# brade31919/radar_depth

Hardware: AMD Instinct MI355X
Metric: training samples/sec, resnet18_latefusion b=16 450x800 rgbd, 1/2/4/8 MI355X (higher is better)
Workload: dtype f32

## Files before the change

radar_depth_amd/csrc/layout.hip:

```cpp
#include "common.h"

namespace rd {

__device__ __forceinline__ int64_t packed_index(int quad, int64_t t, int64_t rows, int64_t row, int64_t ldc, int64_t col) {
    return quad ? ((t * (rows >> 2) + (row >> 2)) * ldc + col) * 4 + (row & 3) : (t * rows + row) * ldc + col;
}
__device__ __forceinline__ int64_t packed_index_bf16(int64_t t, int64_t rows, int64_t row, int64_t ldc, int64_t col) {
    return ((t * (rows >> 3) + (row >> 3)) * ldc + col) * 8 + (row & 7);
}
__global__ void pack_weights_kernel(const float* __restrict__ w, float* __restrict__ packed, int O, int I, int T,
                                    int ldc, int off, int rows_total, int transpose) {
    const int64_t total = (int64_t)O * I * T;
    for (int64_t e = (int64_t)blockIdx.x * blockDim.x + threadIdx.x; e < total; e += (int64_t)gridDim.x * blockDim.x) {
        int t, o, i;
        if (!transpose) {
            o = (int)(e % O);
            const int64_t r = e / O;
            i = (int)(r % I);
            t = (int)(r / I);
            packed[packed_index(1, t, I, i, ldc, off + o)] = w[((int64_t)o * I + i) * T + t];
        } else {
            i = (int)(e % I);
            const int64_t r = e / I;
            o = (int)(r % O);
            t = (int)(r / O);
            packed[packed_index(1, t, rows_total, off + o, ldc, i)] = w[((int64_t)o * I + i) * T + t];
        }
    }
}

__global__ void pack_weights_bf16_kernel(const float* __restrict__ w, __bf16* __restrict__ packed, int O, int I, int T,
                                         int ldc, int off, int rows_total, int transpose) {
    const int64_t total = (int64_t)O * I * T;
    for (int64_t e = (int64_t)blockIdx.x * blockDim.x + threadIdx.x; e < total; e += (int64_t)gridDim.x * blockDim.x) {
        const int o = (int)(e % O);
        const int64_t r = e / O;
        const int i = (int)(r % I), t = (int)(r / I);
        const float v = w[((int64_t)o * I + i) * T + t];
        if (!transpose) packed[packed_index_bf16(t, I, i, ldc, off + o)] = (__bf16)v;
        else packed[packed_index_bf16(t, rows_total, off + o, ldc, i)] = (__bf16)v;
    }
}

struct PackJob {
    const float* src;
    float* dst;
    const float* scale;
    int O, I, T, ldc, off, rows_total, transpose, first_block;
    int quad;
    int scale_col;
};
__device__ __forceinline__ void store_split3(__bf16* dst, int64_t idx, int64_t plane, float v) {
    const __bf16 h = (__bf16)v;
    float r = v - (float)h;
    const __bf16 m = (__bf16)r;
    r -= (float)m;
    dst[idx] = h;
    dst[idx + plane] = m;
    dst[idx + 2 * plane] = (__bf16)r;
}
constexpr int PACK_CHUNK = 2048;
__device__ __forceinline__ void pack_units_bf16(const PackJob& j, int64_t u) {
    const int R = j.transpose ? j.O : j.I;
    const int Cn = j.transpose ? j.I : j.O;
    const int64_t units = (int64_t)(R >> 3) * Cn;
    if (u >= units) return;
    const int col = (int)(u % Cn), r8 = (int)(u / Cn);
    const int rows_total = j.transpose ? j.rows_total : j.I;
    const int row0 = (j.transpose ? j.off : 0) + r8 * 8, colp = (j.transpose ? 0 : j.off) + col;
    __bf16* dst = reinterpret_cast<__bf16*>(j.dst);
    const int64_t plane = (int64_t)j.T * rows_total * j.ldc;
    for (int t = 0; t < j.T; ++t) {
        float v[8];
#pragma unroll
        for (int r = 0; r < 8; ++r) {
            const int o = j.transpose ? r8 * 8 + r : col, i = j.transpose ? col : r8 * 8 + r;
            v[r] = j.src[((int64_t)o * j.I + i) * j.T + t];
            if (j.scale) v[r] *= j.scale[j.scale_col ? i : o];
        }
        const int64_t idx = packed_index_bf16(t, rows_total, row0, j.ldc, colp);
        unsigned w0[4], w1[4], w2[4];
#pragma unroll
        for (int q = 0; q < 4; ++q) {
            float a = v[2 * q], b = v[2 * q + 1];
            w0[q] = cvt_pk_bf16(a, b);
            a -= __uint_as_float(w0[q] << 16); b -= __uint_as_float(w0[q] & 0xffff0000u);
            w1[q] = cvt_pk_bf16(a, b);
            a -= __uint_as_float(w1[q] << 16); b -= __uint_as_float(w1[q] & 0xffff0000u);
            w2[q] = cvt_pk_bf16(a, b);
        }
        *reinterpret_cast<uint4*>(dst + idx) = make_uint4(w0[0], w0[1], w0[2], w0[3]);
        if (j.quad == 3) {
            *reinterpret_cast<uint4*>(dst + idx + plane) = make_uint4(w1[0], w1[1], w1[2], w1[3]);
            *reinterpret_cast<uint4*>(dst + idx + 2 * plane) = make_uint4(w2[0], w2[1], w2[2], w2[3]);
        }
    }
}
__global__ __launch_bounds__(256) void pack_weights_batched_kernel(const PackJob* __restrict__ jobs, const int* __restrict__ block_job) {
    const PackJob j = jobs[block_job[blockIdx.x]];
    if (j.quad >= 2 && ((j.transpose ? (j.O | j.off | j.rows_total) : j.I) & 7) == 0) {
        pack_units_bf16(j, (int64_t)(blockIdx.x - j.first_block) * 256 + threadIdx.x);
        return;
    }
    const int64_t total = (int64_t)j.O * j.I * j.T;
    const int64_t base = (int64_t)(blockIdx.x - j.first_block) * PACK_CHUNK;
#pragma unroll
    for (int u = 0; u < PACK_CHUNK / 256; ++u) {
        const int64_t e64 = base + u * 256 + threadIdx.x;
        if (e64 >= total) break;
        const unsigned e = (unsigned)e64;
        if (!j.transpose) {
            const unsigned r = e / (unsigned)j.O;
            const int o = (int)(e - r * (unsigned)j.O);
            const int t = (int)(r / (unsigned)j.I), i = (int)(r - (r / (unsigned)j.I) * (unsigned)j.I);
            float v = j.src[((int64_t)o * j.I + i) * j.T + t];
            if (j.scale) v *= j.scale[j.scale_col ? i : o];
            if (j.quad == 3) store_split3(reinterpret_cast<__bf16*>(j.dst), packed_index_bf16(t, j.I, i, j.ldc, j.off + o), (int64_t)j.T * j.I * j.ldc, v);
            else if (j.quad == 2) reinterpret_cast<__bf16*>(j.dst)[packed_index_bf16(t, j.I, i, j.ldc, j.off + o)] = (__bf16)v;
            else j.dst[packed_index(j.quad, t, j.I, i, j.ldc, j.off + o)] = v;
        } else {
            const unsigned r = e / (unsigned)j.I;
            const int i = (int)(e - r * (unsigned)j.I);
            const int t = (int)(r / (unsigned)j.O), o = (int)(r - (r / (unsigned)j.O) * (unsigned)j.O);
            float v = j.src[((int64_t)o * j.I + i) * j.T + t];
            if (j.scale) v *= j.scale[j.scale_col ? i : o];
            if (j.quad == 3) store_split3(reinterpret_cast<__bf16*>(j.dst), packed_index_bf16(t, j.rows_total, j.off + o, j.ldc, i), (int64_t)j.T * j.rows_total * j.ldc, v);
            else if (j.quad == 2) reinterpret_cast<__bf16*>(j.dst)[packed_index_bf16(t, j.rows_total, j.off + o, j.ldc, i)] = (__bf16)v;
            else j.dst[packed_index(j.quad, t, j.rows_total, j.off + o, j.ldc, i)] = v;
        }
    }
}

__global__ void fill_kernel(float* __restrict__ p, int64_t n, float v) {
    for (int64_t e = (int64_t)blockIdx.x * blockDim.x + threadIdx.x; e < n; e += (int64_t)gridDim.x * blockDim.x) p[e] = v;
}

__global__ void transpose_kernel(const float* __restrict__ src, float* __restrict__ dst, int rows, int cols) {
    __shared__ float tile[32][33];
    const int n = blockIdx.z;
    src += (size_t)n * rows * cols;
    dst += (size_t)n * rows * cols;
    const int c0 = blockIdx.x * 32, r0 = blockIdx.y * 32;
    for (int j = threadIdx.y; j < 32; j += blockDim.y) {
        const int r = r0 + j, c = c0 + threadIdx.x;
        if (r < rows && c < cols) tile[j][threadIdx.x] = src[(size_t)r * cols + c];
    }
    rd_sync();
    for (int j = threadIdx.y; j < 32; j += blockDim.y) {
        const int c = c0 + j, r = r0 + threadIdx.x;
        if (r < rows && c < cols) dst[(size_t)c * rows + r] = tile[threadIdx.x][j];
    }
}

static int grid_for(int64_t n, int block) {
// ... 81 lines not shown
```

radar_depth_amd/csrc/wgrad.hip:

```cpp
#include <stdlib.h>

#include <mutex>
#include <string>
#include <type_traits>
#include <unordered_map>
#include <vector>

#include "common.h"

namespace rd {

template <int B, int E, int ST, typename F>
__device__ __forceinline__ void static_for(F&& f) {
    if constexpr (B < E) {
        f(std::integral_constant<int, B>{});
        static_for<B + ST, E, ST>(f);
    }
}

constexpr int WG_MAX_TG = 9;
constexpr int WG_MAX_GROUPS = 5;
constexpr int WG_MAX_PIX = 512;
constexpr int WG_PITCH = 27;

struct WgTapGroup {
    int n;
    int8_t dh[WG_MAX_TG], dw[WG_MAX_TG], oh[WG_MAX_TG], ow[WG_MAX_TG];
    int16_t widx[WG_MAX_TG];
};

struct WgradArgs {
    const float* in;
    const float* dout;
    float* slabs;
    int N, Hi, Wi, Cin, ldi, Ho, Wo, Cout, ldo, IS, OS;
    int lh, lw, TH, TW, tiles_h, tiles_w, total_tiles, tiles_per_split, n_splits;
    int dh_min, dh_max, dw_min, dw_max;
    int n_cib, n_cob, n_tg;
    int S;
    int compact, off_h, off_w;
    int debug;
    WgTapGroup tg[WG_MAX_GROUPS];
};

template <int TG, int MF, bool LAYOUT_A, bool SHB, int PITCH, int RW>
__global__ __launch_bounds__(256) __attribute__((amdgpu_waves_per_eu(2))) void wgrad_kernel(const WgradArgs a) {
    constexpr int CIB = LAYOUT_A ? 64 : MF;
    constexpr int COB = LAYOUT_A ? 64 : MF;
    constexpr int KP = MF == 32 ? 2 : 4;
    constexpr int WLP = LAYOUT_A ? 1 : 4;
    constexpr int NACC = MF == 32 ? 16 : 4;
    extern __shared__ __attribute__((aligned(16))) float smem[];
    const int tid = threadIdx.x, lane = tid & 63, wave = tid >> 6;
    const int lm = lane & (MF - 1), lk = lane / MF;
    const int wci = LAYOUT_A ? (wave >> 1) : 0, wco = LAYOUT_A ? (wave & 1) : 0;
    const int wpix = LAYOUT_A ? 0 : wave;

    const int vid = xcd_remap(blockIdx.x, gridDim.x);
    const int n_groups = a.n_cib * a.n_cob * a.n_tg;
    const int g = vid % n_groups, split = vid / n_groups;
    const int tgi = g % a.n_tg;
// ... 300 lines not shown
            _Pragma("unroll") for (int t = 0; t < TG; ++t) acc[t] = __builtin_amdgcn_mfma_f32_32x32x2f32(AV[t], BV, acc[t], 0, 0, 0);
#define RD_WS_SCHED()                                                                              \
            _Pragma("unroll") for (int i = 0; i < TG; ++i) {                                           \
                __builtin_amdgcn_sched_group_barrier(0x008, 1, 0);                                     \
                __builtin_amdgcn_sched_group_barrier(0x100, 1, 0);                                     \
            }                                                                                          \
            __builtin_amdgcn_sched_barrier(0);
            RD_WS_LOAD(a0, b0, 0)
            __builtin_amdgcn_sched_barrier(0);
            static_for<0, 2 * STEPS, 2>([&](auto sc) {
                constexpr int S = decltype(sc)::value;
                RD_WS_LOAD(a1, b1, S + 1)
                RD_WS_MFMA(a0, b0)
                RD_WS_SCHED()
                if constexpr (S + 2 < 2 * STEPS) { RD_WS_LOAD(a0, b0, S + 2) }
                RD_WS_MFMA(a1, b1)
                RD_WS_SCHED()
            });
#undef RD_WS_LOAD
#undef RD_WS_MFMA
#undef RD_WS_SCHED
        }
    }

    float* slab = a.slabs + (size_t)split * a.S * a.Cin * a.Cout;
    const int co = cob0 + wco * 32 + lm;
#pragma unroll
    for (int t = 0; t < TG; ++t) {
        float* dst = slab + (size_t)G.widx[t] * a.Cin * a.Cout;
#pragma unroll
        for (int i = 0; i < 16; ++i) {
            const int ci = cib0 + wci * 32 + (i & 3) + 8 * (i >> 2) + 4 * lk;
            if (ci < a.Cin && co < a.Cout) dst[(size_t)ci * a.Cout + co] = acc[t][i];
        }
    }
}

__global__ __launch_bounds__(256) void wgrad_reduce1_kernel(const float* __restrict__ slabs, float* __restrict__ tmp,
                                                            int n_splits, int J, int64_t E4) {
    const int j = blockIdx.y;
    const float4* src = reinterpret_cast<const float4*>(slabs);
    float4* dst = reinterpret_cast<float4*>(tmp);
    for (int64_t e = (int64_t)blockIdx.x * blockDim.x + threadIdx.x; e < E4; e += (int64_t)gridDim.x * blockDim.x) {
        float4 s = make_float4(0.f, 0.f, 0.f, 0.f);
#pragma unroll 4
        for (int k = j; k < n_splits; k += J) {
            const float4 v = src[(int64_t)k * E4 + e];
            s.x += v.x; s.y += v.y; s.z += v.z; s.w += v.w;
        }
        dst[(int64_t)j * E4 + e] = s;
    }
}

__global__ __launch_bounds__(256) void wgrad_reduce2_kernel(const float* __restrict__ tmp, float* __restrict__ grad, int J,
                                                            int64_t E, int S, int Cin, int Cout, int O, int I, int co_off,
                                                            int accumulate) {
    const int64_t total = (int64_t)S * I * O;
    const bool small = total < (1ll << 31);
    for (int64_t e = (int64_t)blockIdx.x * blockDim.x + threadIdx.x; e < total; e += (int64_t)gridDim.x * blockDim.x) {
        int o, i, t;
        if (small) {
            const unsigned u = (unsigned)e, r = u / (unsigned)O;
            o = (int)(u - r * (unsigned)O);
            t = (int)(r / (unsigned)I);
            i = (int)(r - (unsigned)t * (unsigned)I);
        } else {
            o = (int)(e % O);
            const int64_t r = e / O;
            i = (int)(r % I);
            t = (int)(r / I);
        }
        const float* src = tmp + ((int64_t)t * Cin + i) * Cout + co_off + o;
        float s = 0.f;
        for (int k = 0; k < J; ++k) s += src[k * E];
        float* dst = grad + ((int64_t)o * I + i) * S + t;
        *dst = accumulate ? *dst + s : s;
    }
}

int launch_slab_reduce(const float* slabs, int n_splits, int64_t E, float* tmp, float* grad_oihw, int S, int Cin, int Cout,
                       int O, int I, int co_off, int accumulate, hipStream_t s) {
    RD_CHECK_ARG(E % 4 == 0, "slab_reduce: slab size must be a multiple of 4");
    const int J = n_splits < 16 ? n_splits : 16;
    const int64_t E4 = E / 4;
    if (n_splits <= 16) tmp = const_cast<float*>(slabs);
    else if (co_off == 0) {
        int64_t g1 = cdiv64(E4, 256);
        if (g1 > 2048) g1 = 2048;
        hipLaunchKernelGGL(wgrad_reduce1_kernel, dim3((int)g1, J), dim3(256), 0, s, slabs, tmp, n_splits, J, E4);
        RD_CHECK_LAUNCH("wgrad_reduce1_kernel");
    }
    const int64_t total = (int64_t)S * I * O;
    int64_t g = cdiv64(total, 256);
    if (g > 4096) g = 4096;
    hipLaunchKernelGGL(wgrad_reduce2_kernel, dim3((int)g), dim3(256), 0, s, tmp, grad_oihw, J, E, S, Cin, Cout, O, I, co_off,
                       accumulate);
    RD_CHECK_LAUNCH("wgrad_reduce2_kernel");
    return RD_OK;
}

__global__ __launch_bounds__(256) void wgrad_reduce1_batched_kernel(const RdReduceJob* __restrict__ jobs, const int32_t* __restrict__ block_job) {
    const RdReduceJob jb = jobs[block_job[blockIdx.x]];
    const int lb = (int)blockIdx.x - jb.first_block1;
    const int J = jb.J, j = lb % J, bx = lb / J, nbx = jb.n_blocks1 / J;
    const int64_t E4 = jb.E / 4;
    const float4* src = reinterpret_cast<const float4*>(jb.slabs);
    float4* dst = reinterpret_cast<float4*>(jb.tmp);
    for (int64_t e = (int64_t)bx * 256 + threadIdx.x; e < E4; e += (int64_t)nbx * 256) {
        float4 s = make_float4(0.f, 0.f, 0.f, 0.f);
#pragma unroll 4
        for (int k = j; k < jb.n_splits; k += J) {
            const float4 v = src[(int64_t)k * E4 + e];
            s.x += v.x; s.y += v.y; s.z += v.z; s.w += v.w;
        }
        dst[(int64_t)j * E4 + e] = s;
    }
}

__global__ __launch_bounds__(256) void wgrad_reduce2_batched_kernel(const RdReduceJob* __restrict__ jobs, const int32_t* __restrict__ block_job) {
    const RdReduceJob jb = jobs[block_job[blockIdx.x]];
    const int lb = (int)blockIdx.x - jb.first_block2;
    const unsigned total = (unsigned)jb.S * (unsigned)jb.I * (unsigned)jb.O;
    const float* tmp = jb.n_splits <= 16 ? jb.slabs : jb.tmp;
    for (unsigned u = (unsigned)lb * 256u + threadIdx.x; u < total; u += (unsigned)jb.n_blocks2 * 256u) {
        const unsigned r = u / (unsigned)jb.O;
        const int o = (int)(u - r * (unsigned)jb.O);
        const int t = (int)(r / (unsigned)jb.I);
        const int i = (int)(r - (unsigned)t * (unsigned)jb.I);
        const float* src = tmp + ((int64_t)t * jb.Cin + i) * jb.Cout + jb.co_off + o;
        float s = 0.f;
        for (int k = 0; k < jb.J; ++k) s += src[k * jb.E];
        float* dst = jb.grad + ((int64_t)o * jb.I + i) * jb.S + t;
        *dst = jb.accumulate ? *dst + s : s;
    }
}

int make_reduce_job(const float* slabs, int n_splits, int64_t E, float* grad_oihw, int S, int Cin, int Cout, int O, int I, int co_off,
                    int accumulate, RdReduceJob* jb) {
    RD_CHECK_ARG(E % 4 == 0, "slab_reduce: slab size must be a multiple of 4");
    RD_CHECK_ARG((int64_t)S * I * O < (1ll << 31), "wgrad_reduce_job: one weight tensor must stay below 2^31 elements");
    const int J = n_splits < 16 ? n_splits : 16;
    jb->slabs = slabs; jb->tmp = const_cast<float*>(slabs) + (int64_t)n_splits * E; jb->grad = grad_oihw;
    jb->E = E; jb->n_splits = n_splits; jb->J = J; jb->S = S; jb->Cin = Cin; jb->Cout = Cout; jb->O = O; jb->I = I;
    jb->co_off = co_off; jb->accumulate = accumulate;
    int64_t g1 = cdiv64(E / 4, 256);
    if (g1 > 2048) g1 = 2048;
    jb->n_blocks1 = (n_splits > 16 && co_off == 0) ? (int)g1 * J : 0;
    int64_t g2 = cdiv64((int64_t)S * I * O, 256);
    if (g2 > 4096) g2 = 4096;
    jb->n_blocks2 = (int)g2;
    jb->first_block1 = jb->first_block2 = 0;
    jb->pad_ = 0;
    return RD_OK;
}

struct WgradPlan {
    int TG, MF, layoutA;
    int TH, TW, tiles_h, tiles_w, total_tiles, tiles_per_split, n_splits, slab_splits;
    int n_cib, n_cob, n_tg, S, J, shb;
    int pitch;
    int rw;
    int per_phase;
    int strip;
    int w16;
    int w1x1;
    WgradStripArgs sa;
    size_t lds;
};

static inline bool tile_is_tiled(const struct WgradPlan* tile);
static int plan_wgrad(const RdConvDesc& d_in, WgradPlan& pl, WgradArgs* out, int ph = -1, const WgradPlan* tile = nullptr) {
    RdConvDesc d = d_in;
    int S_all = 0;
    for (int i = 0; i < d_in.n_phases; ++i)
        for (int t = 0; t < d_in.phase[i].n_taps; ++t) S_all = S_all > d_in.phase[i].widx[t] + 1 ? S_all : d_in.phase[i].widx[t] + 1;
    if (ph >= 0) {
        d.n_phases = 1;
        d.phase[0] = d_in.phase[ph];
    }
    const RdPhase& P0 = d.phase[0];
    int ntaps = 0, S = 0;
    int dh_min = 127, dh_max = -127, dw_min = 127, dw_max = -127;
    for (int i = 0; i < d.n_phases; ++i) {
        const RdPhase& p = d.phase[i];
        RD_CHECK_ARG(p.lh == P0.lh && p.lw == P0.lw, "wgrad: phases must share one logical grid");
        ntaps += p.n_taps;
        for (int t = 0; t < p.n_taps; ++t) S = S > p.widx[t] + 1 ? S : p.widx[t] + 1;
        dh_min = dh_min < p.dh_min ? dh_min : p.dh_min;
        dh_max = dh_max > p.dh_max ? dh_max : p.dh_max;
        dw_min = dw_min < p.dw_min ? dw_min : p.dw_min;
        dw_max = dw_max > p.dw_max ? dw_max : p.dw_max;
    }
    S = S_all;
// ... 371 lines not shown
```

radar_depth_amd/csrc/wino_split.hip:

```cpp
#include <stdlib.h>

#include <type_traits>

#include "common.h"

namespace rd {

typedef __bf16 wbf16x8 __attribute__((ext_vector_type(8)));
typedef unsigned int wu32x4 __attribute__((ext_vector_type(4)));
typedef float wf32x2 __attribute__((ext_vector_type(2)));
typedef __bf16 wbf16x2 __attribute__((ext_vector_type(2)));

constexpr int WN_TBH = 4, WN_TBW = 8;
constexpr int WN_T = WN_TBH * WN_TBW;
constexpr int WN_CB = 64;
constexpr int WN_AH = 16 * 3 * 2 * 512;
constexpr int WN_BH = 16 * 3 * 2 * 1024;
constexpr int WN_BUF = WN_AH;
constexpr int WN_ZP = 68;
constexpr unsigned WN_OOB = 0x80000000u;

struct WinoArgs {
    const float* in;
    const unsigned short* u;
// ... 239 lines not shown
            const float4 xv = ld4(a.bnb_x + px * a.bnb_ld + co);
            const float gx = y.x * act_grad_from_out(fmaf(bS.x, xv.x, bT.x), a.bnb_act), gy = y.y * act_grad_from_out(fmaf(bS.y, xv.y, bT.y), a.bnb_act);
            const float gz = y.z * act_grad_from_out(fmaf(bS.z, xv.z, bT.z), a.bnb_act), gw = y.w * act_grad_from_out(fmaf(bS.w, xv.w, bT.w), a.bnb_act);
            ssum.x += gx; ssum.y += gy; ssum.z += gz; ssum.w += gw;
            ssq.x += gx * (xv.x - bM.x); ssq.y += gy * (xv.y - bM.y); ssq.z += gz * (xv.z - bM.z); ssq.w += gw * (xv.w - bM.w);
        } else {
            ssum.x += y.x; ssum.y += y.y; ssum.z += y.z; ssum.w += y.w;
            ssq.x += y.x * y.x; ssq.y += y.y * y.y; ssq.z += y.z * y.z; ssq.w += y.w * y.w;
        }
    };
#pragma unroll
    for (int it = 0; it < 2; ++it) {
        const int rt = (tid >> 4) + 32 * it;
        const int m = rt >> 1, r = rt & 1;
        float4 z[4];
#pragma unroll
        for (int j = 0; j < 4; ++j) z[j] = *reinterpret_cast<const float4*>(zb + ((j * 2 + r) * WN_T + m) * WN_ZP + c4 * 4);
        float4 y0 = make_float4(z[0].x + z[1].x + z[2].x, z[0].y + z[1].y + z[2].y, z[0].z + z[1].z + z[2].z, z[0].w + z[1].w + z[2].w);
        float4 y1 = make_float4(z[1].x - z[2].x - z[3].x, z[1].y - z[2].y - z[3].y, z[1].z - z[2].z - z[3].z, z[1].w - z[2].w - z[3].w);
        const int oy = 2 * (by * WN_TBH + (m >> 3)) + r, ox = 2 * (bx * WN_TBW + (m & 7));
        const bool okr = oy < a.H && co < a.Cout;
        const bool ok0 = okr && ox < a.W, ok1 = okr && ox + 1 < a.W;
        const size_t pix = ((size_t)n * a.H + oy) * a.W + ox;
        if (a.addend) {
            if (ok0) { const float4 v = ld4(a.addend + pix * a.ld_add + co); y0.x += v.x; y0.y += v.y; y0.z += v.z; y0.w += v.w; }
            if (ok1) { const float4 v = ld4(a.addend + (pix + 1) * a.ld_add + co); y1.x += v.x; y1.y += v.y; y1.z += v.z; y1.w += v.w; }
        }
        if (ok0) {
            st4(a.out + pix * a.ldo + co, y0);
            if (a.stat) account(y0, pix);
        }
        if (ok1) {
            st4(a.out + (pix + 1) * a.ldo + co, y1);
            if (a.stat) account(y1, pix + 1);
        }
    }
    if (a.stat) {
        rd_sync();
        float* red = reinterpret_cast<float*>(wsm);
        const int row = tid >> 4;
        *reinterpret_cast<float4*>(red + (row * 2 + 0) * 64 + c4 * 4) = ssum;
        *reinterpret_cast<float4*>(red + (row * 2 + 1) * 64 + c4 * 4) = ssq;
        rd_sync();
        if (tid < 128) {
            const int which = tid >> 6, j = tid & 63;
            float s = 0.f;
#pragma unroll 8
            for (int rw = 0; rw < 32; ++rw) s += red[(rw * 2 + which) * 64 + j];
            if (cot * WN_CB + j < a.Cout) a.stat[((size_t)pt * (bnb ? 3 : 2) + which) * a.Cout + cot * WN_CB + j] = s;
        }
    }
}

__device__ __forceinline__ void wino_pack_body(const float* __restrict__ w, int O, int I, int flip, unsigned short* __restrict__ u, int e) {
    const int R = flip ? O : I, Q = flip ? I : O;
    const int r8n = R >> 3;
    if (e >= Q * r8n) return;
    const int q = e / r8n, r8 = e - q * r8n;
    const int nck = R >> 4;
    const int cot = q >> 6, ql = q & 63;
    const int chunk = r8 >> 1, kh8 = r8 & 1;
    unsigned short pc[16][3][8];
#pragma unroll
    for (int k = 0; k < 8; ++k) {
        const int r = r8 * 8 + k;
        const float* g = flip ? w + ((size_t)r * I + q) * 9 : w + ((size_t)q * I + r) * 9;
        double gg[3][3];
#pragma unroll
        for (int y = 0; y < 3; ++y)
#pragma unroll
            for (int x = 0; x < 3; ++x) gg[y][x] = flip ? (double)g[(2 - y) * 3 + (2 - x)] : (double)g[y * 3 + x];
        double t[4][3];
#pragma unroll
        for (int x = 0; x < 3; ++x) {
            t[0][x] = gg[0][x];
            t[1][x] = 0.5 * (gg[0][x] + gg[1][x] + gg[2][x]);
            t[2][x] = 0.5 * (gg[0][x] - gg[1][x] + gg[2][x]);
            t[3][x] = gg[2][x];
        }
#pragma unroll
        for (int i = 0; i < 4; ++i) {
            const double uu[4] = {t[i][0], 0.5 * (t[i][0] + t[i][1] + t[i][2]), 0.5 * (t[i][0] - t[i][1] + t[i][2]), t[i][2]};
#pragma unroll
            for (int j = 0; j < 4; ++j) {
                float f = (float)uu[j];
                const __bf16 p0 = (__bf16)uu[j];
                f -= (float)p0;
                const __bf16 p1 = (__bf16)f;
                f -= (float)p1;
                const __bf16 p2 = (__bf16)f;
                pc[i * 4 + j][0][k] = __builtin_bit_cast(unsigned short, p0);
                pc[i * 4 + j][1][k] = __builtin_bit_cast(unsigned short, p1);
                pc[i * 4 + j][2][k] = __builtin_bit_cast(unsigned short, p2);
            }
        }
    }
#pragma unroll
    for (int i = 0; i < 4; ++i)
#pragma unroll
        for (int j = 0; j < 4; ++j)
#pragma unroll
            for (int p = 0; p < 3; ++p) {
                const size_t o = ((size_t)cot * nck + chunk) * WN_BH + (((i * 4 + j) * 3 + p) * 2 + kh8) * 1024 + ql * 16;
                uint4 v;
                v.x = pc[i * 4 + j][p][0] | ((unsigned)pc[i * 4 + j][p][1] << 16);
                v.y = pc[i * 4 + j][p][2] | ((unsigned)pc[i * 4 + j][p][3] << 16);
                v.z = pc[i * 4 + j][p][4] | ((unsigned)pc[i * 4 + j][p][5] << 16);
                v.w = pc[i * 4 + j][p][6] | ((unsigned)pc[i * 4 + j][p][7] << 16);
                *reinterpret_cast<uint4*>(reinterpret_cast<char*>(u) + o) = v;
            }
}

__global__ __launch_bounds__(256) void wino_pack_kernel(const float* __restrict__ w, int O, int I, int flip, unsigned short* __restrict__ u) {
    wino_pack_body(w, O, I, flip, u, blockIdx.x * blockDim.x + threadIdx.x);
}

struct WinoPackJob {
    const float* w;
    unsigned short* u;
    int32_t O, I, flip, first_block;
};
__global__ __launch_bounds__(256) void wino_pack_batched_kernel(const WinoPackJob* __restrict__ jobs, const int32_t* __restrict__ block_job) {
    const WinoPackJob j = jobs[block_job[blockIdx.x]];
    wino_pack_body(j.w, j.O, j.I, j.flip, j.u, (blockIdx.x - j.first_block) * blockDim.x + threadIdx.x);
}

static bool wino_shape_ok(int H, int W, int Cin, int Cout, int ldi, int ldo) {
    return H >= 2 && W >= 2 && Cin >= 64 && Cin % 16 == 0 && Cout >= 64 && Cout % 64 == 0 && ldi % 4 == 0 && ldo % 4 == 0 &&
           (long long)H * W * ldi * 4 < 0x7fffffffll;
}
}

extern "C" int64_t rd_wino_packed_bytes(int32_t O, int32_t I, int32_t flip) {
    const int R = flip ? O : I, Q = flip ? I : O;
    return (int64_t)((Q + 63) / 64) * (R / 16) * rd::WN_BH;
}

extern "C" int rd_wino_pack(const float* w_oihw, int32_t O, int32_t I, int32_t flip, void* u_packed, void* stream) {
    RD_CHECK_ARG(w_oihw && u_packed && O > 0 && I > 0, "rd_wino_pack: bad arguments");
    const int R = flip ? O : I, Q = flip ? I : O;
    RD_CHECK_ARG(R % 16 == 0 && Q % 64 == 0, "rd_wino_pack: reduction channels %d %% 16, output channels %d %% 64", R, Q);
    const int n = Q * (R / 8);
    hipLaunchKernelGGL(rd::wino_pack_kernel, dim3((n + 255) / 256), dim3(256), 0, static_cast<hipStream_t>(stream), w_oihw, O, I, flip,
                       static_cast<unsigned short*>(u_packed));
    RD_CHECK_LAUNCH("wino_pack_kernel");
    return RD_OK;
}

extern "C" int rd_wino_pack_blocks(int32_t O, int32_t I, int32_t flip) {
    const int R = flip ? O : I, Q = flip ? I : O;
    return (Q * (R / 8) + 255) / 256;
}
extern "C" int rd_wino_pack_batched(const void* jobs, const int32_t* block_job, int32_t n_blocks, void* stream) {
    RD_CHECK_ARG(jobs && block_job && n_blocks > 0, "rd_wino_pack_batched: bad arguments");
    static_assert(sizeof(rd::WinoPackJob) == 32, "job record layout");
    hipLaunchKernelGGL(rd::wino_pack_batched_kernel, dim3(n_blocks), dim3(256), 0, static_cast<hipStream_t>(stream),
                       static_cast<const rd::WinoPackJob*>(jobs), block_job);
    RD_CHECK_LAUNCH("wino_pack_batched_kernel");
    return RD_OK;
}

extern "C" int rd_wino_preferred(int32_t H, int32_t W, int32_t Cin, int32_t Cout, int32_t ldi, int32_t ldo) {
    if (!rd::wino_shape_ok(H, W, Cin, Cout, ldi, ldo)) return 0;
    static const char* env = getenv("RD_WINO");
    if (env && !strcmp(env, "0")) return 0;
    if (env && !strcmp(env, "all")) return 1;
    return (Cin >= 512 || ((long long)H * W <= 1536 && Cin <= 128)) ? 1 : 0;
}

extern "C" int rd_wino_supported(int32_t H, int32_t W, int32_t Cin, int32_t Cout, int32_t ldi, int32_t ldo) {
    return rd::wino_shape_ok(H, W, Cin, Cout, ldi, ldo) ? 1 : 0;
}

extern "C" int rd_wino_stat_tiles(int32_t N, int32_t H, int32_t W) {
    const int th = (H + 1) / 2, tw = (W + 1) / 2;
    return N * ((th + rd::WN_TBH - 1) / rd::WN_TBH) * ((tw + rd::WN_TBW - 1) / rd::WN_TBW);
}
// ... 52 lines not shown
```

Before: 1103.

## Stage OIHW weight reads and gradient writes through LDS for coalesced access

Weight packing, the Winograd weight pack and the weight-gradient slab reduction now stage contiguous OIHW runs through shared memory tiles instead of scattered per-element global loads and stores. Reads and writes become vectorised float4 runs along the contiguous dimension, and a shared tile-shape helper picks tile sizes per tap count. This targets the uncoalesced memory traffic in the per-step weight packing and wgrad finalisation, at the cost of extra block barriers, LDS use and more complex boundary handling.

```diff
diff --git a/radar_depth_amd/csrc/layout.hip b/radar_depth_amd/csrc/layout.hip
--- a/radar_depth_amd/csrc/layout.hip
+++ b/radar_depth_amd/csrc/layout.hip
@@ -1,4 +1,5 @@
 #include "common.h"
+#include "oihw_tiles.h"
 
 namespace rd {
 
@@ -60,46 +61,79 @@
     dst[idx + 2 * plane] = (__bf16)r;
 }
 constexpr int PACK_CHUNK = 2048;
-__device__ __forceinline__ void pack_units_bf16(const PackJob& j, int64_t u) {
-    const int R = j.transpose ? j.O : j.I;
+__device__ __forceinline__ void pack_units_bf16(const PackJob& j, const PackTile& pt, int lb, int nb, float* lds) {
+#pragma clang fp contract(off)
+    const int tid = threadIdx.x;
+    const int R8 = (j.transpose ? j.O : j.I) >> 3;
     const int Cn = j.transpose ? j.I : j.O;
-    const int64_t units = (int64_t)(R >> 3) * Cn;
-    if (u >= units) return;
-    const int col = (int)(u % Cn), r8 = (int)(u / Cn);
+    const int n_ct = (Cn + pt.co - 1) / pt.co, n_kt = (R8 + pt.k8 - 1) / pt.k8;
     const int rows_total = j.transpose ? j.rows_total : j.I;
-    const int row0 = (j.transpose ? j.off : 0) + r8 * 8, colp = (j.transpose ? 0 : j.off) + col;
     __bf16* dst = reinterpret_cast<__bf16*>(j.dst);
     const int64_t plane = (int64_t)j.T * rows_total * j.ldc;
-    for (int t = 0; t < j.T; ++t) {
-        float v[8];
-#pragma unroll
-        for (int r = 0; r < 8; ++r) {
-            const int o = j.transpose ? r8 * 8 + r : col, i = j.transpose ? col : r8 * 8 + r;
-            v[r] = j.src[((int64_t)o * j.I + i) * j.T + t];
-            if (j.scale) v[r] *= j.scale[j.scale_col ? i : o];
-        }
-        const int64_t idx = packed_index_bf16(t, rows_total, row0, j.ldc, colp);
-        unsigned w0[4], w1[4], w2[4];
-#pragma unroll
-        for (int q = 0; q < 4; ++q) {
-            float a = v[2 * q], b = v[2 * q + 1];
-            w0[q] = cvt_pk_bf16(a, b);
-            a -= __uint_as_float(w0[q] << 16); b -= __uint_as_float(w0[q] & 0xffff0000u);
-            w1[q] = cvt_pk_bf16(a, b);
-            a -= __uint_as_float(w1[q] << 16); b -= __uint_as_float(w1[q] & 0xffff0000u);
-            w2[q] = cvt_pk_bf16(a, b);
-        }
-        *reinterpret_cast<uint4*>(dst + idx) = make_uint4(w0[0], w0[1], w0[2], w0[3]);
-        if (j.quad == 3) {
-            *reinterpret_cast<uint4*>(dst + idx + plane) = make_uint4(w1[0], w1[1], w1[2], w1[3]);
-            *reinterpret_cast<uint4*>(dst + idx + 2 * plane) = make_uint4(w2[0], w2[1], w2[2], w2[3]);
+    const int T = j.T, LP = pt.lp;
+    for (int tile = lb; tile < n_ct * n_kt; tile += nb) {
+        if (tile != lb) rd_sync();
+        const int kt = tile / n_ct, ct = tile - kt * n_ct;
+        const int c0 = ct * pt.co, u0 = kt * pt.k8;
+        const int cn = Cn - c0 < pt.co ? Cn - c0 : pt.co, kn = R8 - u0 < pt.k8 ? R8 - u0 : pt.k8;
+        const int n_runs = j.transpose ? kn * 8 : cn, len = j.transpose ? cn * T : kn * 8 * T;
+        const int nq = (len + 6) >> 2;
+        for (int idx = tid; idx < n_runs * nq; idx += 256) {
+            const int r = idx / nq, q = idx - r * nq;
+            const float* run = j.src + (j.transpose ? ((int64_t)(u0 * 8 + r) * j.I + c0) * T : ((int64_t)(c0 + r) * j.I + u0 * 8) * T);
+            const int a = (int)((reinterpret_cast<uintptr_t>(run) >> 2) & 3);
+            const int c = 4 * q - a;
+            if (c >= len) continue;
+            float* l = lds + r * LP + c;
+            if (c >= 0 && c + 4 <= len) {
+                const float4 v = *reinterpret_cast<const float4*>(run + c);
+                l[0] = v.x; l[1] = v.y; l[2] = v.z; l[3] = v.w;
+            } else {
+#pragma unroll
+                for (int e = 0; e < 4; ++e)
+                    if (c + e >= 0 && c + e < len) l[e] = run[c + e];
+            }
+        }
+        rd_sync();
+        for (int item = tid; item < cn * kn * T; item += 256) {
+            const int col = item % cn, kt_ = item / cn;
+            const int k = kt_ / T, t = kt_ - k * T;
+            float v[8];
+#pragma unroll
+            for (int r = 0; r < 8; ++r) {
+                v[r] = j.transpose ? lds[(k * 8 + r) * LP + col * T + t] : lds[col * LP + (k * 8 + r) * T + t];
+                if (j.scale) {
+                    const int o = j.transpose ? (u0 + k) * 8 + r : c0 + col, i = j.transpose ? c0 + col : (u0 + k) * 8 + r;
+                    v[r] *= j.scale[j.scale_col ? i : o];
+                }
+            }
+            const int row0 = (j.transpose ? j.off : 0) + (u0 + k) * 8, colp = (j.transpose ? 0 : j.off) + c0 + col;
+            const int64_t idx = packed_index_bf16(t, rows_total, row0, j.ldc, colp);
+            unsigned w0[4], w1[4], w2[4];
+#pragma unroll
+            for (int q = 0; q < 4; ++q) {
+                float a = v[2 * q], b = v[2 * q + 1];
+                w0[q] = cvt_pk_bf16(a, b);
+                a -= __uint_as_float(w0[q] << 16); b -= __uint_as_float(w0[q] & 0xffff0000u);
+                w1[q] = cvt_pk_bf16(a, b);
+                a -= __uint_as_float(w1[q] << 16); b -= __uint_as_float(w1[q] & 0xffff0000u);
+                w2[q] = cvt_pk_bf16(a, b);
+            }
+            *reinterpret_cast<uint4*>(dst + idx) = make_uint4(w0[0], w0[1], w0[2], w0[3]);
+            if (j.quad == 3) {
+                *reinterpret_cast<uint4*>(dst + idx + plane) = make_uint4(w1[0], w1[1], w1[2], w1[3]);
+                *reinterpret_cast<uint4*>(dst + idx + 2 * plane) = make_uint4(w2[0], w2[1], w2[2], w2[3]);
+            }
         }
     }
 }
 __global__ __launch_bounds__(256) void pack_weights_batched_kernel(const PackJob* __restrict__ jobs, const int* __restrict__ block_job) {
+    __shared__ float lds[PACK_LDS];
     const PackJob j = jobs[block_job[blockIdx.x]];
-    if (j.quad >= 2 && ((j.transpose ? (j.O | j.off | j.rows_total) : j.I) & 7) == 0) {
-        pack_units_bf16(j, (int64_t)(blockIdx.x - j.first_block) * 256 + threadIdx.x);
+    const PackTile pt = pack_tile(j.T, j.transpose);
+    if (j.quad >= 2 && ((j.transpose ? (j.O | j.off | j.rows_total) : j.I) & 7) == 0 && pt.co > 0) {
+        const int nb = (int)(((int64_t)j.O * j.I * j.T + PACK_CHUNK - 1) / PACK_CHUNK);
+        pack_units_bf16(j, pt, (int)(blockIdx.x - j.first_block), nb, lds);
         return;
     }
     const int64_t total = (int64_t)j.O * j.I * j.T;
diff --git a/radar_depth_amd/csrc/oihw_tiles.h b/radar_depth_amd/csrc/oihw_tiles.h
--- /dev/null
+++ b/radar_depth_amd/csrc/oihw_tiles.h
@@ -0,0 +1,45 @@
+#pragma once
+#include <cstdint>
+
+#if defined(__HIPCC__)
+#define RD_TILE_FN __host__ __device__ inline
+#else
+#define RD_TILE_FN inline
+#endif
+
+namespace rd {
+
+constexpr int RED_TO = 32;
+constexpr int RED_MAX_S = 64;
+constexpr int RED_RUN = 80;
+constexpr int RED_LDS = RED_TO * (RED_RUN + 1);
+struct RedTile { int to, ti, n_ob, n_ib; };
+RD_TILE_FN RedTile red_tile(int S, int I, int O) {
+    RedTile r;
+    r.ti = (32 + S - 1) / S;
+    if (r.ti > I) r.ti = I;
+    r.to = RED_TO;
+    const int64_t tiles = (int64_t)((O + RED_TO - 1) / RED_TO) * ((I + r.ti - 1) / r.ti);
+    if (tiles < 256) r.to = RED_TO / 2;
+    else if (tiles >= 2048 && 2 * r.ti * S <= RED_RUN && 2 * r.ti <= I) r.ti *= 2;
+    r.n_ob = (O + r.to - 1) / r.to;
+    r.n_ib = (I + r.ti - 1) / r.ti;
+    return r;
+}
+
+constexpr int PACK_LDS = 6656;
+struct PackTile { int co, k8, lp; };
+RD_TILE_FN PackTile pack_tile(int T, int transpose) {
+    PackTile p;
+    p.co = 0; p.k8 = 1; p.lp = 1;
+    if (T < 1 || T > 1024) return p;
+    p.k8 = T >= 4 ? 1 : (T == 1 ? 4 : 2);
+    for (p.co = 64; p.co >= 8; p.co >>= 1) {
+        p.lp = (transpose ? p.co * T : p.k8 * 8 * T) | 1;
+        if ((int64_t)(transpose ? p.k8 * 8 : p.co) * p.lp <= PACK_LDS && (p.co <= 32 || T <= 9)) return p;
+    }
+    p.co = 0;
+    return p;
+}
+
+}
diff --git a/radar_depth_amd/csrc/wgrad.hip b/radar_depth_amd/csrc/wgrad.hip
--- a/radar_depth_amd/csrc/wgrad.hip
+++ b/radar_depth_amd/csrc/wgrad.hip
@@ -7,6 +7,7 @@
 #include <vector>
 
 #include "common.h"
+#include "oihw_tiles.h"
 
 namespace rd {
 
@@ -413,35 +414,93 @@
     }
 }
 
+__device__ __forceinline__ void reduce2_tile(const float* __restrict__ tmp, float* __restrict__ grad, int J, int64_t E, int S, int Cin,
+                                             int Cout, int O, int I, int co_off, int accumulate, const RedTile& rt, int64_t tile,
+                                             float* lds) {
+    const int tid = threadIdx.x;
+    const int ob = (int)(tile / rt.n_ib), ib = (int)(tile - (int64_t)ob * rt.n_ib);
+    const int o0 = ob * rt.to, i0 = ib * rt.ti;
+    const int ton = O - o0 < rt.to ? O - o0 : rt.to, tin = I - i0 < rt.ti ? I - i0 : rt.ti;
+    const int rows = tin * S, LP = (rt.ti * S) | 1;
+    if (((Cout | co_off) & 3) == 0 && (reinterpret_cast<uintptr_t>(tmp) & 15) == 0) {
+        const int lpr = rt.to >> 2, oq = (tid % lpr) * 4;
+        if (oq < ton) {
+            for (int rr = tid / lpr; rr < rows; rr += 256 / lpr) {
+                const int t = rr / tin, il = rr - t * tin;
+                const float* src = tmp + ((int64_t)t * Cin + i0 + il) * Cout + co_off + o0 + oq;
+                float4 s = make_float4(0.f, 0.f, 0.f, 0.f);
+                int k = 0;
+                for (; k + 4 <= J; k += 4) {
+                    float4 v[4];
+#pragma unroll
+                    for (int x = 0; x < 4; ++x) v[x] = *reinterpret_cast<const float4*>(src + (k + x) * E);
+#pragma unroll
+                    for (int x = 0; x < 4; ++x) { s.x += v[x].x; s.y += v[x].y; s.z += v[x].z; s.w += v[x].w; }
+                }
+                for (; k < J; ++k) {
+                    const float4 v = *reinterpret_cast<const float4*>(src + k * E);
+                    s.x += v.x; s.y += v.y; s.z += v.z; s.w += v.w;
+                }
+                float* d = lds + oq * LP + il * S + t;
+                d[0] = s.x;
+                if (oq + 1 < ton) d[LP] = s.y;
+                if (oq + 2 < ton) d[2 * LP] = s.z;
+                if (oq + 3 < ton) d[3 * LP] = s.w;
+            }
+        }
+    } else {
+        const int ol = tid % rt.to;
+        if (ol < ton) {
+            for (int rr = tid / rt.to; rr < rows; rr += 256 / rt.to) {
+                const int t = rr / tin, il = rr - t * tin;
+                const float* src = tmp + ((int64_t)t * Cin + i0 + il) * Cout + co_off + o0 + ol;
+                float s = 0.f;
+                for (int k = 0; k < J; ++k) s += src[k * E];
+                lds[ol * LP + il * S + t] = s;
+            }
+        }
+    }
+    rd_sync();
+    const int nq = (rows + 6) >> 2;
+    for (int idx = tid; idx < ton * nq; idx += 256) {
+        const int r = idx / nq, q = idx - r * nq;
+        float* run = grad + ((int64_t)(o0 + r) * I + i0) * S;
+        const int a = (int)((reinterpret_cast<uintptr_t>(run) >> 2) & 3);
+        const int c = 4 * q - a;
+        if (c >= rows) continue;
+        const float* l = lds + r * LP + c;
+        if (c >= 0 && c + 4 <= rows) {
+            float4 s = make_float4(l[0], l[1], l[2], l[3]);
+            float4* dst = reinterpret_cast<float4*>(run + c);
+            if (accumulate) {
+                const float4 d = *dst;
+                s.x = d.x + s.x; s.y = d.y + s.y; s.z = d.z + s.z; s.w = d.w + s.w;
+            }
+            *dst = s;
+        } else {
+#pragma unroll
+            for (int e = 0; e < 4; ++e)
+                if (c + e >= 0 && c + e < rows) run[c + e] = accumulate ? run[c + e] + l[e] : l[e];
+        }
+    }
+}
+
 __global__ __launch_bounds__(256) void wgrad_reduce2_kernel(const float* __restrict__ tmp, float* __restrict__ grad, int J,
                                                             int64_t E, int S, int Cin, int Cout, int O, int I, int co_off,
                                                             int accumulate) {
-    const int64_t total = (int64_t)S * I * O;
-    const bool small = total < (1ll << 31);
-    for (int64_t e = (int64_t)blockIdx.x * blockDim.x + threadIdx.x; e < total; e += (int64_t)gridDim.x * blockDim.x) {
-        int o, i, t;
-        if (small) {
-            const unsigned u = (unsigned)e, r = u / (unsigned)O;
-            o = (int)(u - r * (unsigned)O);
-            t = (int)(r / (unsigned)I);
-            i = (int)(r - (unsigned)t * (unsigned)I);
-        } else {
-            o = (int)(e % O);
-            const int64_t r = e / O;
-            i = (int)(r % I);
-            t = (int)(r / I);
-        }
-        const float* src = tmp + ((int64_t)t * Cin + i) * Cout + co_off + o;
-        float s = 0.f;
-        for (int k = 0; k < J; ++k) s += src[k * E];
-        float* dst = grad + ((int64_t)o * I + i) * S + t;
-        *dst = accumulate ? *dst + s : s;
+    __shared__ float lds[RED_LDS];
+    const RedTile rt = red_tile(S, I, O);
+    const int64_t tiles = (int64_t)rt.n_ob * rt.n_ib;
+    for (int64_t tile = blockIdx.x; tile < tiles; tile += gridDim.x) {
+        if (tile != (int64_t)blockIdx.x) rd_sync();
+        reduce2_tile(tmp, grad, J, E, S, Cin, Cout, O, I, co_off, accumulate, rt, tile, lds);
     }
 }
 
 int launch_slab_reduce(const float* slabs, int n_splits, int64_t E, float* tmp, float* grad_oihw, int S, int Cin, int Cout,
                        int O, int I, int co_off, int accumulate, hipStream_t s) {
     RD_CHECK_ARG(E % 4 == 0, "slab_reduce: slab size must be a multiple of 4");
+    RD_CHECK_ARG(S > 0 && S <= RED_MAX_S && O > 0 && I > 0, "slab_reduce: %d taps, %d x %d channels unsupported", S, O, I);
     const int J = n_splits < 16 ? n_splits : 16;
     const int64_t E4 = E / 4;
     if (n_splits <= 16) tmp = const_cast<float*>(slabs);
@@ -451,9 +510,9 @@
         hipLaunchKernelGGL(wgrad_reduce1_kernel, dim3((int)g1, J), dim3(256), 0, s, slabs, tmp, n_splits, J, E4);
         RD_CHECK_LAUNCH("wgrad_reduce1_kernel");
     }
-    const int64_t total = (int64_t)S * I * O;
-    int64_t g = cdiv64(total, 256);
-    if (g > 4096) g = 4096;
+    const RedTile rt = red_tile(S, I, O);
+    int64_t g = (int64_t)rt.n_ob * rt.n_ib;
+    if (g > (1 << 20)) g = 1 << 20;
     hipLaunchKernelGGL(wgrad_reduce2_kernel, dim3((int)g), dim3(256), 0, s, tmp, grad_oihw, J, E, S, Cin, Cout, O, I, co_off,
                        accumulate);
     RD_CHECK_LAUNCH("wgrad_reduce2_kernel");
@@ -479,20 +538,15 @@
 }
 
 __global__ __launch_bounds__(256) void wgrad_reduce2_batched_kernel(const RdReduceJob* __restrict__ jobs, const int32_t* __restrict__ block_job) {
+    __shared__ float lds[RED_LDS];
     const RdReduceJob jb = jobs[block_job[blockIdx.x]];
     const int lb = (int)blockIdx.x - jb.first_block2;
-    const unsigned total = (unsigned)jb.S * (unsigned)jb.I * (unsigned)jb.O;
     const float* tmp = jb.n_splits <= 16 ? jb.slabs : jb.tmp;
-    for (unsigned u = (unsigned)lb * 256u + threadIdx.x; u < total; u += (unsigned)jb.n_blocks2 * 256u) {
-        const unsigned r = u / (unsigned)jb.O;
-        const int o = (int)(u - r * (unsigned)jb.O);
-        const int t = (int)(r / (unsigned)jb.I);
-        const int i = (int)(r - (unsigned)t * (unsigned)jb.I);
-        const float* src = tmp + ((int64_t)t * jb.Cin + i) * jb.Cout + jb.co_off + o;
-        float s = 0.f;
-        for (int k = 0; k < jb.J; ++k) s += src[k * jb.E];
-        float* dst = jb.grad + ((int64_t)o * jb.I + i) * jb.S + t;
-        *dst = jb.accumulate ? *dst + s : s;
+    const RedTile rt = red_tile(jb.S, jb.I, jb.O);
+    const int tiles = rt.n_ob * rt.n_ib;
+    for (int tile = lb; tile < tiles; tile += jb.n_blocks2) {
+        if (tile != lb) rd_sync();
+        reduce2_tile(tmp, jb.grad, jb.J, jb.E, jb.S, jb.Cin, jb.Cout, jb.O, jb.I, jb.co_off, jb.accumulate, rt, tile, lds);
     }
 }
 
@@ -500,6 +554,7 @@
                     int accumulate, RdReduceJob* jb) {
     RD_CHECK_ARG(E % 4 == 0, "slab_reduce: slab size must be a multiple of 4");
     RD_CHECK_ARG((int64_t)S * I * O < (1ll << 31), "wgrad_reduce_job: one weight tensor must stay below 2^31 elements");
+    RD_CHECK_ARG(S > 0 && S <= RED_MAX_S && O > 0 && I > 0, "wgrad_reduce_job: %d taps, %d x %d channels unsupported", S, O, I);
     const int J = n_splits < 16 ? n_splits : 16;
     jb->slabs = slabs; jb->tmp = const_cast<float*>(slabs) + (int64_t)n_splits * E; jb->grad = grad_oihw;
     jb->E = E; jb->n_splits = n_splits; jb->J = J; jb->S = S; jb->Cin = Cin; jb->Cout = Cout; jb->O = O; jb->I = I;
diff --git a/radar_depth_amd/csrc/wino_split.hip b/radar_depth_amd/csrc/wino_split.hip
--- a/radar_depth_amd/csrc/wino_split.hip
+++ b/radar_depth_amd/csrc/wino_split.hip
@@ -315,49 +315,88 @@
     }
 }
 
-__device__ __forceinline__ void wino_pack_body(const float* __restrict__ w, int O, int I, int flip, unsigned short* __restrict__ u, int e) {
+constexpr int WP_PITCH0 = 4 * 9 + 1, WP_PITCH1 = 64 * 9 + 1;
+constexpr int WP_WAVE = 64 * WP_PITCH0;
+static_assert(4 * WP_PITCH1 <= WP_WAVE, "wino_pack: LDS of a wave");
+__device__ __forceinline__ void wino_pack_body(const float* __restrict__ w, int O, int I, int flip, unsigned short* __restrict__ u, int e,
+                                               float* lds_block) {
     const int R = flip ? O : I, Q = flip ? I : O;
     const int r8n = R >> 3;
-    if (e >= Q * r8n) return;
-    const int q = e / r8n, r8 = e - q * r8n;
     const int nck = R >> 4;
-    const int cot = q >> 6, ql = q & 63;
+    const int lane = threadIdx.x & 63, rest = e >> 6;
+    const bool valid = rest < (Q >> 6) * r8n;
+    const int cot = rest / r8n, r8 = rest - cot * r8n;
+    const int ql = lane;
     const int chunk = r8 >> 1, kh8 = r8 & 1;
-    unsigned short pc[16][3][8];
-#pragma unroll
-    for (int k = 0; k < 8; ++k) {
-        const int r = r8 * 8 + k;
-        const float* g = flip ? w + ((size_t)r * I + q) * 9 : w + ((size_t)q * I + r) * 9;
-        double gg[3][3];
-#pragma unroll
-        for (int y = 0; y < 3; ++y)
-#pragma unroll
-            for (int x = 0; x < 3; ++x) gg[y][x] = flip ? (double)g[(2 - y) * 3 + (2 - x)] : (double)g[y * 3 + x];
-        double t[4][3];
-#pragma unroll
-        for (int x = 0; x < 3; ++x) {
-            t[0][x] = gg[0][x];
-            t[1][x] = 0.5 * (gg[0][x] + gg[1][x] + gg[2][x]);
-            t[2][x] = 0.5 * (gg[0][x] - gg[1][x] + gg[2][x]);
-            t[3][x] = gg[2][x];
-        }
-#pragma unroll
-        for (int i = 0; i < 4; ++i) {
-            const double uu[4] = {t[i][0], 0.5 * (t[i][0] + t[i][1] + t[i][2]), 0.5 * (t[i][0] - t[i][1] + t[i][2]), t[i][2]};
-#pragma unroll
-            for (int j = 0; j < 4; ++j) {
-                float f = (float)uu[j];
-                const __bf16 p0 = (__bf16)uu[j];
-                f -= (float)p0;
-                const __bf16 p1 = (__bf16)f;
-                f -= (float)p1;
-                const __bf16 p2 = (__bf16)f;
-                pc[i * 4 + j][0][k] = __builtin_bit_cast(unsigned short, p0);
-                pc[i * 4 + j][1][k] = __builtin_bit_cast(unsigned short, p1);
-                pc[i * 4 + j][2][k] = __builtin_bit_cast(unsigned short, p2);
+    float* lds = lds_block + (threadIdx.x >> 6) * WP_WAVE;
+    unsigned pc[16][3][4];
+#pragma unroll
+    for (int h = 0; h < 2; ++h) {
+        if (h) rd_sync();
+        if (valid) {
+            const int n_runs = flip ? 4 : 64, len = flip ? 64 * 9 : 4 * 9, pitch = flip ? WP_PITCH1 : WP_PITCH0;
+            const int nq = (len + 6) >> 2;
+            for (int idx = lane; idx < n_runs * nq; idx += 64) {
+                const int rr = idx / nq, qq = idx - rr * nq;
+                const float* run = flip ? w + ((size_t)(r8 * 8 + 4 * h + rr) * I + cot * 64) * 9
+                                        : w + ((size_t)(cot * 64 + rr) * I + r8 * 8 + 4 * h) * 9;
+                const int a = (int)((reinterpret_cast<uintptr_t>(run) >> 2) & 3);
+                const int c = 4 * qq - a;
+                if (c >= len) continue;
+                float* l = lds + rr * pitch + c;
+                if (c >= 0 && c + 4 <= len) {
+                    const float4 v = *reinterpret_cast<const float4*>(run + c);
+                    l[0] = v.x; l[1] = v.y; l[2] = v.z; l[3] = v.w;
+                } else {
+#pragma unroll
+                    for (int x = 0; x < 4; ++x)
+                        if (c + x >= 0 && c + x < len) l[x] = run[c + x];
+                }
+            }
+        }
+        rd_sync();
+        if (valid) {
+#pragma unroll
+            for (int kk = 0; kk < 4; ++kk) {
+                const int k = 4 * h + kk;
+                const float* g = flip ? lds + kk * WP_PITCH1 + ql * 9 : lds + ql * WP_PITCH0 + kk * 9;
+                double gg[3][3];
+#pragma unroll
+                for (int y = 0; y < 3; ++y)
+#pragma unroll
+                    for (int x = 0; x < 3; ++x) gg[y][x] = flip ? (double)g[(2 - y) * 3 + (2 - x)] : (double)g[y * 3 + x];
+                double t[4][3];
+#pragma unroll
+                for (int x = 0; x < 3; ++x) {
+                    t[0][x] = gg[0][x];
+                    t[1][x] = 0.5 * (gg[0][x] + gg[1][x] + gg[2][x]);
+                    t[2][x] = 0.5 * (gg[0][x] - gg[1][x] + gg[2][x]);
+                    t[3][x] = gg[2][x];
+                }
+#pragma unroll
+                for (int i = 0; i < 4; ++i) {
+                    const double uu[4] = {t[i][0], 0.5 * (t[i][0] + t[i][1] + t[i][2]), 0.5 * (t[i][0] - t[i][1] + t[i][2]), t[i][2]};
+#pragma unroll
+                    for (int j = 0; j < 4; ++j) {
+                        float f = (float)uu[j];
+                        const __bf16 p0 = (__bf16)uu[j];
+                        f -= (float)p0;
+                        const __bf16 p1 = (__bf16)f;
+                        f -= (float)p1;
+                        const __bf16 p2 = (__bf16)f;
+                        const unsigned b0 = __builtin_bit_cast(unsigned short, p0), b1 = __builtin_bit_cast(unsigned short, p1),
+                                       b2 = __builtin_bit_cast(unsigned short, p2);
+                        if (k & 1) {
+                            pc[i * 4 + j][0][k >> 1] |= b0 << 16; pc[i * 4 + j][1][k >> 1] |= b1 << 16; pc[i * 4 + j][2][k >> 1] |= b2 << 16;
+                        } else {
+                            pc[i * 4 + j][0][k >> 1] = b0; pc[i * 4 + j][1][k >> 1] = b1; pc[i * 4 + j][2][k >> 1] = b2;
+                        }
+                    }
+                }
             }
         }
     }
+    if (!valid) return;
 #pragma unroll
     for (int i = 0; i < 4; ++i)
 #pragma unroll
@@ -365,17 +404,14 @@
 #pragma unroll
             for (int p = 0; p < 3; ++p) {
                 const size_t o = ((size_t)cot * nck + chunk) * WN_BH + (((i * 4 + j) * 3 + p) * 2 + kh8) * 1024 + ql * 16;
-                uint4 v;
-                v.x = pc[i * 4 + j][p][0] | ((unsigned)pc[i * 4 + j][p][1] << 16);
-                v.y = pc[i * 4 + j][p][2] | ((unsigned)pc[i * 4 + j][p][3] << 16);
-                v.z = pc[i * 4 + j][p][4] | ((unsigned)pc[i * 4 + j][p][5] << 16);
-                v.w = pc[i * 4 + j][p][6] | ((unsigned)pc[i * 4 + j][p][7] << 16);
-                *reinterpret_cast<uint4*>(reinterpret_cast<char*>(u) + o) = v;
+                *reinterpret_cast<uint4*>(reinterpret_cast<char*>(u) + o) =
+                    make_uint4(pc[i * 4 + j][p][0], pc[i * 4 + j][p][1], pc[i * 4 + j][p][2], pc[i * 4 + j][p][3]);
             }
 }
 
 __global__ __launch_bounds__(256) void wino_pack_kernel(const float* __restrict__ w, int O, int I, int flip, unsigned short* __restrict__ u) {
-    wino_pack_body(w, O, I, flip, u, blockIdx.x * blockDim.x + threadIdx.x);
+    __shared__ float lds[4 * WP_WAVE];
+    wino_pack_body(w, O, I, flip, u, blockIdx.x * blockDim.x + threadIdx.x, lds);
 }
 
 struct WinoPackJob {
@@ -385,7 +421,8 @@
 };
 __global__ __launch_bounds__(256) void wino_pack_batched_kernel(const WinoPackJob* __restrict__ jobs, const int32_t* __restrict__ block_job) {
     const WinoPackJob j = jobs[block_job[blockIdx.x]];
-    wino_pack_body(j.w, j.O, j.I, j.flip, j.u, (blockIdx.x - j.first_block) * blockDim.x + threadIdx.x);
+    __shared__ float lds[4 * WP_WAVE];
+    wino_pack_body(j.w, j.O, j.I, j.flip, j.u, (blockIdx.x - j.first_block) * blockDim.x + threadIdx.x, lds);
 }
 
 static bool wino_shape_ok(int H, int W, int Cin, int Cout, int ldi, int ldo) {
```

Result: no change. 1114 (median of 6 runs) (+1.0%).
